# bowang-lab/BioReason

Measured on AMD Instinct MI355X. Metric: GRPO samples/sec (NT-500M+Qwen3-1.7B, DNA 2x1024, prompt 2180, gen 256), higher is better.
Workload: dtype bf16

## Files before the change

bioreason_amd/csrc/k_wgrad.hip:

```cpp
#include "bra_device.h"
#include "bra_api_internal.h"
#include "bra_lora_plan.h"

namespace bra {

struct WgradArgs {
    const bf16_t* Y; long ldy;
    const bf16_t* T; long ldt;
    float* C; long c_sn, c_sr;
    int M, N, R;
    int m_chunk;
    float alpha;
    DropCfg d;
    int nb_live;
};

constexpr int WG_YP = 128 + 8;

template <int RB, int DROP, int NL = RB, int RM = 0, int TR = 32, int NT = NL>
__global__ __launch_bounds__(256) void wgrad_tn_kernel(WgradArgs g) {
    static_assert(!DROP || (NL == (NT * TR + 31) / 32 && NT <= 4), "live blocks = the blocks the targets cover");
    constexpr int NYS = DROP ? NT : 2;
    __shared__ bf16_t ys[NYS][32 * WG_YP];
    constexpr int WG_TP = 32 * RB + 8, TPT = RB >= 2 ? RB / 2 : 1;
    __shared__ bf16_t ts[2][32 * WG_TP];
    const int tid = (int)threadIdx.x, lane = tid & 63, wave = tid >> 6, h = lane >> 5;
    const int n0 = (int)blockIdx.x * 128;
    const int m_lo = (int)blockIdx.y * g.m_chunk;
    int m_hi = m_lo + g.m_chunk;
    m_hi = m_hi < g.M ? m_hi : g.M;
    const int nstep = m_hi > m_lo ? (m_hi - m_lo + 31) / 32 : 0;
    const u32x4 zero4 = {0u, 0u, 0u, 0u};

    const int yr = tid >> 4, yc = (tid & 15) * 8;
    const bool ycol_ok = n0 + yc + 8 <= g.N;
    u32x4 ry[2], rt[TPT];
    auto issue = [&](int s) {
        const int m0 = m_lo + 32 * s;
#pragma unroll
        for (int i = 0; i < 2; ++i) {
            const int m = m0 + yr + 16 * i;
            const int mc = m < g.M ? m : g.M - 1;
            ry[i] = ld16(g.Y + (long)mc * g.ldy + (ycol_ok ? n0 + yc : 0));
        }
#pragma unroll
        for (int i = 0; i < TPT; ++i) {
            const int c = tid + 256 * i, tr = c / (4 * RB), tc = (c % (4 * RB)) * 8;
            const int m = m0 + (tr < 32 ? tr : 0);
            const int mc = m < g.M ? m : g.M - 1;
            rt[i] = ld16(g.T + (long)mc * g.ldt + tc);
        }
    };
    auto commit = [&](int buf, int s) {
        const int m0 = m_lo + 32 * s;
        u32x4 yv[2];
#pragma unroll
        for (int i = 0; i < 2; ++i) yv[i] = (m0 + yr + 16 * i < m_hi && ycol_ok) ? ry[i] : zero4;
        if (DROP) {
#pragma unroll
            for (int i = 0; i < 2; ++i) {
                const uint32_t e0 = (uint32_t)(m_lo + 32 * s + yr + 16 * i) * (uint32_t)g.N + (uint32_t)(n0 + yc);
#pragma unroll
                for (int jt = 0; jt < NT; ++jt)
                    st16(&ys[jt][(yr + 16 * i) * WG_YP + yc], drop_apply8(yv[i], g.d.seed[jt], e0, g.d.thr16, g.d.inv_keep));
            }
        } else {
            st16(&ys[buf][yr * WG_YP + yc], yv[0]);
            st16(&ys[buf][(yr + 16) * WG_YP + yc], yv[1]);
        }
#pragma unroll
        for (int i = 0; i < TPT; ++i) {
            const int c = tid + 256 * i, tr = c / (4 * RB), tc = (c % (4 * RB)) * 8;
            const int m = m0 + (tr < 32 ? tr : 0);
            if (tr < 32) st16(&ts[buf][tr * WG_TP + tc], m < m_hi ? rt[i] : zero4);
        }
    };

    f32x16 acc[RB];
#pragma unroll
    for (int rb = 0; rb < RB; ++rb)
#pragma unroll
        for (int r = 0; r < 16; ++r) acc[rb][r] = 0.f;

    if (nstep > 0) { issue(0); commit(0, 0); }
    __syncthreads();
    const int ncol0 = wave * 32 + (lane & 31);
    constexpr bool r_major = RM != 0;
    for (int s = 0; s < nstep; ++s) {
        const int buf = s & 1;
        issue(s + 1 < nstep ? s + 1 : s);
        sched_fence();
        const int ncol = opaque_i(ncol0);
#pragma unroll
        for (int kk = 0; kk < 2; ++kk) {
            const int mb = 16 * kk + 8 * h;
            u32x4 af0;
            if (!DROP) {
#pragma unroll
                for (int j = 0; j < 4; ++j)
                    af0[j] = (uint32_t)ys[buf][(mb + 2 * j) * WG_YP + ncol] | ((uint32_t)ys[buf][(mb + 2 * j + 1) * WG_YP + ncol] << 16);
            }
            auto y_frag = [&](int jt) {
                u32x4 f;
#pragma unroll
                for (int j = 0; j < 4; ++j)
                    f[j] = (uint32_t)ys[jt][(mb + 2 * j) * WG_YP + ncol] | ((uint32_t)ys[jt][(mb + 2 * j + 1) * WG_YP + ncol] << 16);
                return f;
            };
            auto t_frag = [&](int rb) {
                const int rc = rb * 32 + (lane & 31);
                uint32_t b[4];
#pragma unroll
                for (int j = 0; j < 4; ++j)
                    b[j] = (uint32_t)ts[buf][(mb + 2 * j) * WG_TP + rc] | ((uint32_t)ts[buf][(mb + 2 * j + 1) * WG_TP + rc] << 16);
                const u32x4 bf = {b[0], b[1], b[2], b[3]};
                return bf;
            };
            if constexpr (!DROP || TR == 32) {
#pragma unroll
                for (int rb = 0; rb < NL; ++rb) {
                    u32x4 af = af0;
                    if (DROP) af = y_frag(rb);
                    const u32x4 bf = t_frag(rb);
                    acc[rb] = r_major ? mfma_32x32x16(bf, af, acc[rb]) : mfma_32x32x16(af, bf, acc[rb]);
                }
            } else if constexpr (TR > 32) {
#pragma unroll
                for (int jt = 0; jt < NT; ++jt) {
                    const u32x4 af = y_frag(jt);
#pragma unroll
                    for (int b = 0; b < TR / 32; ++b) {
                        const int rb = jt * (TR / 32) + b;
                        const u32x4 bf = t_frag(rb);
                        acc[rb] = r_major ? mfma_32x32x16(bf, af, acc[rb]) : mfma_32x32x16(af, bf, acc[rb]);
                    }
                }
            } else {
#pragma unroll
                for (int jt = 0; jt < NT; ++jt) {
                    const int rb = jt * TR / 32;
                    const u32x4 af = y_frag(jt);
                    const u32x4 tf = t_frag(rb);
                    const u32x4 bf = (lane & 31) / TR == jt % (32 / TR) ? tf : zero4;
                    acc[rb] = r_major ? mfma_32x32x16(bf, af, acc[rb]) : mfma_32x32x16(af, bf, acc[rb]);
                }
            }
        }
        if (DROP) __syncthreads();
        if (s + 1 < nstep) commit(buf ^ 1, s + 1);
        __syncthreads();
    }
    if (nstep == 0) return;
    if (r_major) {
        const int n = n0 + wave * 32 + (lane & 31);
        float* const cb = g.C + (long)n * g.c_sn + (long)(4 * h) * g.c_sr;
#pragma unroll
        for (int rb = 0; rb < RB; ++rb)
#pragma unroll
            for (int q = 0; q < 16; ++q) {
                const int rq = rb * 32 + (q & 3) + 8 * (q >> 2);
                if (n < g.N && rq + 4 * h < g.R) atomicAdd(cb + (long)rq * g.c_sr, g.alpha * acc[rb][q]);
            }
        return;
    }
    float* const cb = g.C + (long)(n0 + wave * 32 + 4 * h) * g.c_sn + (long)(lane & 31) * g.c_sr;
#pragma unroll
    for (int rb = 0; rb < RB; ++rb) {
        const int r = rb * 32 + (lane & 31);
        if (r >= g.R) continue;
#pragma unroll
        for (int q = 0; q < 16; ++q) {
            const int nq = (q & 3) + 8 * (q >> 2);
            const int n = n0 + wave * 32 + nq + 4 * h;
            if (n < g.N) atomicAdd(cb + (long)nq * g.c_sn + (long)(32 * rb) * g.c_sr, g.alpha * acc[rb][q]);
        }
    }
}

}

using namespace bra;

static int wgrad_launch(WgradArgs& g, int m_chunk, bool drop, const LoraSlice& s, void* stream) {
    if (m_chunk <= 0) {
        const int ntile = (g.N + 127) / 128;
        int splits = (512 + ntile - 1) / ntile;
        m_chunk = (g.M + splits - 1) / splits;
        m_chunk = m_chunk < 256 ? 256 : m_chunk;
    }
    g.m_chunk = (m_chunk + 31) / 32 * 32;
    const dim3 grid((g.N + 127) / 128, (g.M + g.m_chunk - 1) / g.m_chunk);
    bra_stream_t st = (bra_stream_t)stream;
    const bool rm = g.c_sn == 1;
#define BRA_WG(C_, RB_, NL_, TR_, NT_)                                                                             \
    if (C_) {                                                                                                      \
        if (drop && rm) BRA_LAUNCH((wgrad_tn_kernel<RB_, 1, NL_, 1, TR_, NT_>), grid, dim3(256), 0, st, g);        \
        else if (drop) BRA_LAUNCH((wgrad_tn_kernel<RB_, 1, NL_, 0, TR_, NT_>), grid, dim3(256), 0, st, g);         \
        else if (rm) BRA_LAUNCH((wgrad_tn_kernel<RB_, 0, RB_, 1>), grid, dim3(256), 0, st, g);                     \
        else BRA_LAUNCH((wgrad_tn_kernel<RB_, 0, RB_, 0>), grid, dim3(256), 0, st, g);                             \
    } else
    BRA_LORA_ROWS(BRA_WG) return BRA_ERR_ARG;
#undef BRA_WG
    return BRA_LAUNCH_STATUS();
}

static int wgrad_slices(const void* Y, long ldy, const void* T, long ldt, float* C, long c_sn, long c_sr, int M, int N, int R, float alpha,
                        int m_chunk, bool drop, float p, const unsigned* seeds, int r, int nt, void* stream) {
    return lora_for_slices(r, nt, R, [&](LoraSlice s) {
        if (!drop) { s.r = 32; s.nts = s.Rs / 32; }
        WgradArgs g = {(const bf16_t*)Y, ldy, (const bf16_t*)T + s.c0, ldt, C + (long)s.c0 * c_sr, c_sn, c_sr, M, N, s.Rs, 0, alpha,
                       drop ? make_cfg(p, seeds + s.j0, s.nts) : DropCfg{}, 0};
        return wgrad_launch(g, m_chunk, drop, s, stream);
    });
}

extern "C" int bra_wgrad_tn(const void* Y, long ldy, const void* T, long ldt, float* C, long c_sn, long c_sr, int M, int N,
                            int R, float alpha, int m_chunk, void* stream) {
    if (M == 0 || N == 0) return 0;
    if (!Y || !T || !C || M < 0 || N < 0 || N % 8 || ldy % 8 || ldt % 8 || R <= 0 || (R != 32 && R % 64)) return BRA_ERR_ARG;
    return wgrad_slices(Y, ldy, T, ldt, C, c_sn, c_sr, M, N, R, alpha, m_chunk, false, 0.f, nullptr, 0, 0, stream);
}

extern "C" int bra_wgrad_tn_drop(const void* Y, long ldy, const void* T, long ldt, float* C, long c_sn, long c_sr, int M,
                                 int N, int R, float alpha, int m_chunk, float p, unsigned s0, unsigned s1, unsigned s2,
                                 unsigned s3, int r, int nt, void* stream) {
    if (M == 0 || N == 0) return 0;
    if (!Y || !T || !C || M < 0 || N < 0 || N % 8 || ldy % 8 || ldt % 8 || !lora_drop_ok(p, M, N, r, nt, R)) return BRA_ERR_ARG;
    const unsigned seeds[4] = {s0, s1, s2, s3};
    return wgrad_slices(Y, ldy, T, ldt, C, c_sn, c_sr, M, N, R, alpha, m_chunk, true, p, seeds, r, nt, stream);
}
```

bioreason_amd/engine.py:

```python
from __future__ import annotations

import math
from dataclasses import dataclass, field
from typing import Dict, List, Optional, Tuple

import torch

from . import ops
from .arena import TrainableArena

BF16 = torch.bfloat16


def rope_tables(npos: int, hd: int, theta: float, device, round_bf16: bool = True) -> Tuple[torch.Tensor, torch.Tensor]:
    inv = 1.0 / (theta ** (torch.arange(0, hd, 2, dtype=torch.float32) / hd))
    fr = torch.arange(npos, dtype=torch.float32)[:, None] * inv[None, :]
    c, s = fr.cos(), fr.sin()
    if round_bf16:
        c, s = c.to(BF16).float(), s.to(BF16).float()
    return c.contiguous().to(device), s.contiguous().to(device)


class LoraGroup:

# ... 68 lines not shown


def _mix32(a: int, b: int) -> int:
    h = (a * 0x9E3779B1 + b * 0x85EBCA6B + 0x165667B1) & 0xFFFFFFFF
    h ^= h >> 15
    h = (h * 0x2C1B3C6D) & 0xFFFFFFFF
    h ^= h >> 12
    h = (h * 0x297A2D39) & 0xFFFFFFFF
    h ^= h >> 15
    return h


import contextlib as _contextlib
import os as _os
FUSE_SWIGLU = _os.environ.get("BRA_FUSE_SWIGLU", "1") == "1"

_nullctx = _contextlib.nullcontext

LORA_GROUP_INDEX = {"qkv": 0, "o": 1, "gu": 2, "d": 3}


def lora_drop_seeds(pass_seed: int, layer: int, group: str, n_targets: int):
    base = (layer * 4 + LORA_GROUP_INDEX[group]) * 4
    return [_mix32(pass_seed, base + j) for j in range(n_targets)]


class QwenEngine:
    def __init__(self, cfg, device):
        self.cfg = cfg
        self.device = device
        self.H = cfg.hidden_size
        self.Hq, self.Hkv, self.hd = cfg.num_attention_heads, cfg.num_key_value_heads, cfg.head_dim
        self.F = cfg.intermediate_size
        self.L = cfg.num_hidden_layers
        self.V = cfg.vocab_size
        self.eps = cfg.rms_norm_eps
        self.Nq, self.Nkv = self.Hq * self.hd, self.Hkv * self.hd
        self.scale = self.hd ** -0.5
        self.layers: List[QwenLayerW] = [QwenLayerW() for _ in range(self.L)]
        self.norm_w: torch.Tensor = None
        self.E: torch.Tensor = None
        self.ET: Optional[torch.Tensor] = None
        self._rope = None
        self._rope_len = 0
        self.layer_done_hook = None

    def rope(self, npos: int):
        if self._rope is None or self._rope_len < npos:
            n = max(npos, 512)
            theta = self.cfg.rope_parameters["rope_theta"] if hasattr(self.cfg, "rope_parameters") else self.cfg.rope_theta
            self._rope = rope_tables(n, self.hd, theta, self.device)
            self._rope_len = n
        return self._rope

    def ensure_transposed(self):
        for L in self.layers:
            if L.WqkvT is None:
                L.WqkvT = ops.transpose2d(L.Wqkv)
                L.WoT = ops.transpose2d(L.Wo)
                L.WguT = ops.transpose2d(L.Wgu)
                L.WdT = ops.transpose2d(L.Wd)
        if self.ET is None:
            self.ET = ops.transpose2d(self.E)

    SMALL_M = 8192

    @staticmethod
    def _down(x2d, A, scaling, live_rows):
        if x2d.shape[0] < QwenEngine.SMALL_M and A.shape[0] in (32, 64, 128):
            return ops.lora_down_drop(x2d, A, scaling, 0.0, [0] * min(A.shape[0] // 32, (live_rows + 31) // 32), rank=32)
        return ops.gemm_nt(x2d, A, alpha=scaling)

    @staticmethod
    def _lora_fwd(x2d, W, G: Optional[LoraGroup], on: bool, res=None, out=None, drop=None):
        if G is not None and on:
            if drop is not None:
                t = ops.lora_down_drop(x2d, G.A, G.scaling, drop[0], drop[1], drop[2])
            else:
                t = QwenEngine._down(x2d, G.A, G.scaling, len(G.n_sizes) * G.r)
            return ops.gemm_nt(x2d, W, a2=t, b2=G.B, res=res, out=out), t
        return ops.gemm_nt(x2d, W, res=res, out=out), None

    @staticmethod
    def _lora_bwd(dy, WT, G: Optional[LoraGroup], on: bool, x2d, t, drop=None):
        if G is not None and on:
            dts = QwenEngine._down(dy, G.BT, G.scaling, len(G.n_sizes) * G.r)
            if drop is not None:
                dxl = ops.lora_up_drop(dts, G.AT, drop[0], drop[1], drop[2])
                dx = ops.gemm_nt(dy, WT, res=dxl)
            else:
                dx = ops.gemm_nt(dy, WT, a2=dts, b2=G.AT)
            ops.wgrad_tn(dy, t, G.B_grad)
            ops.wgrad_tn(x2d, dts, G.A_grad, transposed_out=True, drop=drop[:2] if drop is not None else None,
                         rank=drop[2] if drop is not None else 32)
            return dx
        return ops.gemm_nt(dy, WT)

    def _drop(self, m: "SeqMeta", li: int, group: str):
        G = self.layers[li].lora[group]
        if G is None or not m.lora_on or m.drop_p <= 0.0:
            return None
        if G.r not in ops.LORA_DROP_RANKS:
            raise NotImplementedError(f"LoRA dropout needs an adapter rank in {list(ops.LORA_DROP_RANKS)} (one mask stream per target "
                                      f"module, built for these ranks), not r = {G.r}")
        return (m.drop_p, lora_drop_seeds(m.drop_seed, li, group, len(G.n_sizes)), G.r)

    def use_fp8(self, W8):
        eng = self

        class _Ctx:
            def __enter__(self_):
                self_.prev = getattr(eng, "_fp8", None)
                eng._fp8 = W8

            def __exit__(self_, *a):
                eng._fp8 = self_.prev
        return _Ctx()

    def fp8_supported(self) -> bool:
        return self.H % 128 == 0 and self.F % 128 == 0 and self.Nq % 128 == 0

    def fp8_weight_images(self, merged=None):
        out = []
        for li, L in enumerate(self.layers):
            W = merged[li] if merged is not None else {"Wqkv": L.Wqkv, "Wo": L.Wo, "Wgu": L.Wgu, "Wd": L.Wd}
            out.append({"Wqkv": ops.quant_rows_fp8(W["Wqkv"], colw=L.ln1), "Wo": ops.quant_rows_fp8(W["Wo"]),
                        "Wgu": ops.quant_rows_fp8(W["Wgu"], colw=L.ln2), "Wd": ops.quant_rows_fp8(W["Wd"])})
        return out

    def _layer_fwd_fp8(self, li: int, x: torch.Tensor, m: SeqMeta, kv_out, R):
        L = self.layers[li]
        B, S, T = m.B, m.S, m.B * m.S
        cosT, sinT = self.rope(m.max_pos or m.S)
        xq, xs = ops.quant_rows_fp8(x, rms_eps=self.eps)
        qkv = ops.gemm_fp8_nt(xq, xs, R["Wqkv"][0], R["Wqkv"][1])
        q = torch.empty((B, S, self.Hq, self.hd), dtype=BF16, device=x.device)
        if kv_out is None:
            k = torch.empty((B, S, self.Hkv, self.hd), dtype=BF16, device=x.device)
            v = torch.empty((B, S, self.Hkv, self.hd), dtype=BF16, device=x.device)
            s_off = 0
        else:
            kc, vc, s_off = kv_out[:3]
            k, v = kc.permute(0, 2, 1, 3), vc.permute(0, 2, 1, 3)
        ops.qk_norm_rope_fwd(qkv, L.qn, L.kn, cosT, sinT, m.pos, S, self.Hq, self.Hkv, self.hd, self.eps, 1.0, q, k, v, s_off)
        if kv_out is not None:
            k, v = k[:, :s_off + S], v[:, :s_off + S]
        vt = ops.head_transpose(v)
        if kv_out is not None and len(kv_out) > 3 and kv_out[3] is not None:
            kv_out[3].append(vt)
        o, _ = ops.attn_fwd(q, k, vt, m.kmask, True, self.scale, need_lse=False)
        oq, os_ = ops.quant_rows_fp8(o.view(T, self.Nq))
        h = ops.gemm_fp8_nt(oq, os_, R["Wo"][0], R["Wo"][1], res=x)
        hq, hs = ops.quant_rows_fp8(h, rms_eps=self.eps)
        gu = ops.gemm_fp8_nt(hq, hs, R["Wgu"][0], R["Wgu"][1])
        aq, as_ = ops.swiglu_quant_fp8(gu)
        return ops.gemm_fp8_nt(aq, as_, R["Wd"][0], R["Wd"][1], res=h)

    def layer_fwd(self, li: int, x: torch.Tensor, m: SeqMeta, save: bool, kv_out=None):
        w8 = getattr(self, "_fp8", None)
        if w8 is not None and not save:
            return self._layer_fwd_fp8(li, x, m, kv_out, w8[li]), None
        L = self.layers[li]
        B, S, T = m.B, m.S, m.B * m.S
        cosT, sinT = self.rope(m.max_pos or m.S)
        xn = ops.rmsnorm_fwd(x, L.ln1, self.eps)
        qkv, t1 = self._lora_fwd(xn, L.Wqkv, L.lora["qkv"], m.lora_on, drop=self._drop(m, li, "qkv"))
        q = torch.empty((B, S, self.Hq, self.hd), dtype=BF16, device=x.device)
        if kv_out is None:
            k = torch.empty((B, S, self.Hkv, self.hd), dtype=BF16, device=x.device)
            v = torch.empty((B, S, self.Hkv, self.hd), dtype=BF16, device=x.device)
            s_off = 0
        else:
            kc, vc, s_off = kv_out[:3]
            k, v = kc.permute(0, 2, 1, 3), vc.permute(0, 2, 1, 3)
        ops.qk_norm_rope_fwd(qkv, L.qn, L.kn, cosT, sinT, m.pos, S, self.Hq, self.Hkv, self.hd, self.eps, 1.0, q, k, v, s_off)
        if kv_out is not None:
            k, v = k[:, :s_off + S], v[:, :s_off + S]
        vt = ops.head_transpose(v)
        if kv_out is not None and len(kv_out) > 3 and kv_out[3] is not None:
            kv_out[3].append(vt)
        o, lse = ops.attn_fwd(q, k, vt, m.kmask, True, self.scale, need_lse=save)
        o2 = o.view(T, self.Nq)
        h, t2 = self._lora_fwd(o2, L.Wo, L.lora["o"], m.lora_on, res=x, drop=self._drop(m, li, "o"))
        hn = ops.rmsnorm_fwd(h, L.ln2, self.eps)
        gu = t3 = act = None
        if not save and FUSE_SWIGLU:
            G3, d3 = L.lora["gu"], self._drop(m, li, "gu")
            if G3 is not None and m.lora_on:
                t3 = ops.lora_down_drop(hn, G3.A, G3.scaling, d3[0], d3[1], d3[2]) if d3 is not None else self._down(hn, G3.A, G3.scaling, len(G3.n_sizes) * G3.r)
                act = ops.gemm_swiglu(hn, L.Wgu, a2=t3, b2=G3.B)
            else:
                act = ops.gemm_swiglu(hn, L.Wgu)
        if act is None:
            if t3 is not None:
                gu = ops.gemm_nt(hn, L.Wgu, a2=t3, b2=L.lora["gu"].B)
            else:
                gu, t3 = self._lora_fwd(hn, L.Wgu, L.lora["gu"], m.lora_on, drop=self._drop(m, li, "gu"))
            act = ops.swiglu_fwd(gu)
        y, t4 = self._lora_fwd(act, L.Wd, L.lora["d"], m.lora_on, res=h, drop=self._drop(m, li, "d"))
        saved = (x, xn, t1, qkv, q, k, v, o, lse, t2, h, hn, t3, gu, act, t4) if save else None
        return y, saved

    def layer_bwd(self, li: int, dy: torch.Tensor, saved, m: SeqMeta, prefix: int = 0, extra_dkv=None):
        L = self.layers[li]
        (x, xn, t1, qkv, q, k, v, o, lse, t2, h, hn, t3, gu, act, t4) = saved
        B, S, T = m.B, m.S, m.B * m.S
        cosT, sinT = self.rope(m.max_pos or m.S)
        on = m.lora_on
        dact = self._lora_bwd(dy, L.WdT, L.lora["d"], on, act, t4, drop=self._drop(m, li, "d"))
        dgu = ops.swiglu_bwd(gu, dact)
        dhn = self._lora_bwd(dgu, L.WguT, L.lora["gu"], on, hn, t3, drop=self._drop(m, li, "gu"))
        dh = ops.rmsnorm_bwd(dhn, h, L.ln2, self.eps, dres=dy)
        do = self._lora_bwd(dh, L.WoT, L.lora["o"], on, o.view(T, self.Nq), t2, drop=self._drop(m, li, "o"))
        dq, dk, dv = ops.attn_bwd(q, k, v, o, do.view(B, S, self.Hq, self.hd), lse, m.kmask, True, self.scale)
        pre = None
        if prefix > 0:
            pre = (dk[:, :prefix], dv[:, :prefix])
            dk, dv = dk[:, prefix:], dv[:, prefix:]
        if extra_dkv is not None:
            dk = ops.group_sum(extra_dkv[0], extra_dkv[2], add=dk)
            dv = ops.group_sum(extra_dkv[1], extra_dkv[2], add=dv)
        dqkv = ops.qk_norm_rope_bwd(qkv, L.qn, L.kn, cosT, sinT, m.pos, S, self.Hq, self.Hkv, self.hd, self.eps, 1.0, dq, dk, dv)
        dxn = self._lora_bwd(dqkv, L.WqkvT, L.lora["qkv"], on, xn, t1, drop=self._drop(m, li, "qkv"))
        dx = ops.rmsnorm_bwd(dxn, x, L.ln1, self.eps, dres=dh)
        return (dx, pre) if prefix > 0 else dx

    def forward_hidden(self, x: torch.Tensor, m: SeqMeta, save: bool):
        tape = []
        for li in range(self.L):
            x, saved = self.layer_fwd(li, x, m, save)
            tape.append(saved)
        hid = ops.rmsnorm_fwd(x, self.norm_w, self.eps)
        return hid, (tape, x) if save else None

    def backward_hidden(self, dhid: torch.Tensor, tape_x, m: SeqMeta):
        tape, xlast = tape_x
        dx = ops.rmsnorm_bwd(dhid, xlast, self.norm_w, self.eps)
        for li in reversed(range(self.L)):
            dx = self.layer_bwd(li, dx, tape[li], m)
            tape[li] = None
            if self.layer_done_hook is not None:
                self.layer_done_hook(li)
        return dx


    def forward_hidden_shared(self, xp: torch.Tensor, mp: SeqMeta, xc: torch.Tensor, mc: SeqMeta, copies: int, save: bool, side=None):
        R, P, B, C = mp.B, mp.S, mc.B, mc.S
        assert B == R * copies
        dev = xp.device
        tape_p, tape_c = [], []
        main = torch.cuda.current_stream(dev) if side is not None else None
        if side is not None:
            side.wait_stream(main)
            xc.record_stream(side)
        for li in range(self.L):
            kc_r = torch.empty((R, self.Hkv, P, self.hd), dtype=BF16, device=dev)
            vc_r = torch.empty((R, self.Hkv, P, self.hd), dtype=BF16, device=dev)
            xp, sp = self.layer_fwd(li, xp, mp, save, kv_out=(kc_r, vc_r, 0))
            tape_p.append(sp)
            if side is not None:
                ev = torch.cuda.Event()
                ev.record(main)
                kc_r.record_stream(side)
                vc_r.record_stream(side)
            with (torch.cuda.stream(side) if side is not None else _nullctx()):
                if side is not None:
                    side.wait_event(ev)
                kc = torch.empty((B, self.Hkv, P + C, self.hd), dtype=BF16, device=dev)
                vc = torch.empty((B, self.Hkv, P + C, self.hd), dtype=BF16, device=dev)
                ops.group_broadcast(kc_r, kc, copies)
                ops.group_broadcast(vc_r, vc, copies)
                xc, sc = self.layer_fwd(li, xc, mc, save, kv_out=(kc, vc, P))
                tape_c.append(sc)
        last = torch.arange(R, device=dev, dtype=torch.int32) * P + (P - 1)
        xp_last = ops.gather_rows(last, xp)
        hid_last = ops.rmsnorm_fwd(xp_last, self.norm_w, self.eps)
        with (torch.cuda.stream(side) if side is not None else _nullctx()):
            hid_c = ops.rmsnorm_fwd(xc, self.norm_w, self.eps)
        if side is not None:
            main.wait_stream(side)
            for t_ in (hid_c, xc):
                t_.record_stream(main)
        return hid_last, hid_c, ((tape_p, tape_c, xp_last, xc, last) if save else None)

    def backward_hidden_shared(self, dhid_last: torch.Tensor, dhid_c: torch.Tensor, tape, mp: SeqMeta, mc: SeqMeta, copies: int, side=None):
        tape_p, tape_c, xp_last, xc, last = tape
        dev = dhid_c.device
        main = torch.cuda.current_stream(dev) if side is not None else None
        if side is not None:
            side.wait_stream(main)
            dhid_c.record_stream(side)
        with (torch.cuda.stream(side) if side is not None else _nullctx()):
            dxc = ops.rmsnorm_bwd(dhid_c, xc, self.norm_w, self.eps)
        dxp = ops.scatter_rows(last, ops.rmsnorm_bwd(dhid_last, xp_last, self.norm_w, self.eps), mp.B * mp.S)
        for li in reversed(range(self.L)):
            with (torch.cuda.stream(side) if side is not None else _nullctx()):
                dxc, pre = self.layer_bwd(li, dxc, tape_c[li], mc, prefix=mp.S)
                tape_c[li] = None
                if side is not None:
                    ev = torch.cuda.Event()
                    ev.record(side)
            if side is not None:
                main.wait_event(ev)
                pre[0].record_stream(main)
                pre[1].record_stream(main)
            dxp = self.layer_bwd(li, dxp, tape_p[li], mp, extra_dkv=(pre[0], pre[1], copies))
            tape_p[li] = None
# ... 72 lines not shown
```

bioreason_amd/ops.py:

```python
from __future__ import annotations

import math
import os
from typing import Optional, Tuple

import torch

from ._lib import current_stream, get_lib

BF16 = torch.bfloat16


def _ld(t: torch.Tensor) -> int:
    assert t.stride(-1) == 1, "last dim must be contiguous"
    return t.stride(-2) if t.dim() >= 2 else t.shape[-1]


def _rows(t: torch.Tensor) -> int:
    return t.numel() // t.shape[-1]


def _as2d(t: torch.Tensor) -> torch.Tensor:
    return t.reshape(-1, t.shape[-1]) if t.dim() != 2 else t


def gemm_nt(
    a: torch.Tensor,
    b: torch.Tensor,
    *,
    a2: Optional[torch.Tensor] = None,
    b2: Optional[torch.Tensor] = None,
    bias: Optional[torch.Tensor] = None,
    res: Optional[torch.Tensor] = None,
    out: Optional[torch.Tensor] = None,
    alpha: float = 1.0,
    out_f32: bool = False,
    accumulate: bool = False,
) -> torch.Tensor:
    a = _as2d(a)
    M, K = a.shape
    N = b.shape[0]
    assert b.shape[1] == K and a.dtype == BF16 and b.dtype == BF16
    K2 = 0
    if a2 is not None:
        a2 = _as2d(a2)
        K2 = a2.shape[1]
        assert b2 is not None and b2.shape == (N, K2) and a2.shape[0] == M
    if out is None:
        out = torch.empty((M, N), dtype=torch.float32 if out_f32 else BF16, device=a.device)
    else:
        assert out.shape == (M, N) and out.dtype == (torch.float32 if out_f32 else BF16)
    if res is not None:
        res = _as2d(res)
        assert res.shape == (M, N) and res.dtype == BF16
    prof = GEMM_PROFILE
    timed = prof is not None and a.is_cuda and prof.wants(M, N, K, K2)
    if timed:
        e0 = torch.cuda.Event(enable_timing=True)
        e0.record()
    get_lib().call(
        "bra_gemm_bf16_nt", a, _ld(a), b, _ld(b), a2, _ld(a2) if a2 is not None else 0, b2,
        _ld(b2) if b2 is not None else 0, K2, out, _ld(out), M, N, K, alpha, bias, res,
        _ld(res) if res is not None else 0, int(out_f32), int(accumulate), current_stream(a),
    )
    if timed:
        e1 = torch.cuda.Event(enable_timing=True)
        e1.record()
        nbytes = 2.0 * (M * K + N * K + (M + N) * K2 + (M * N if res is not None else 0)) + M * N * (4.0 if out_f32 else 2.0)
        prof.records.append((2.0 * M * N * (K + K2), e0, e1, nbytes, (M, N, K, K2, res is not None)))
    return out


class GemmProfile:

    def __init__(self, min_m: int = 1024, dominant_only: bool = True):
        self.min_m = min_m
        self.dominant_only = dominant_only
        self.records = []

    def wants(self, M: int, N: int, K: int, K2: int) -> bool:
        if not self.dominant_only:
            return M >= self.min_m
        if K % 64 or K2 % 64:
            return False
        t = ((M + 255) // 256) * ((N + 255) // 256)
        rounds = (t + 255) // 256
        if t >= 140 and (t <= 256 or 100 * t >= 75 * rounds * 256):
            return True
        if ((M + 255) // 256) * ((N + 127) // 128) >= 128:
            return True
        return ((M + 127) // 128) * ((N + 127) // 128) >= 128

    def summary(self):
        torch.cuda.synchronize()
        fl = sum(r[0] for r in self.records)
        ms = sum(r[1].elapsed_time(r[2]) for r in self.records)
        n = len(self.records)
        by = sum(r[3] for r in self.records)
        return {"launches": n, "flops": fl, "ms": ms, "avg_launch_ms": ms / max(n, 1), "tflops": fl / max(ms, 1e-9) / 1e9,
                "flops_per_launch": fl / max(n, 1), "bytes_per_launch": by / max(n, 1)}


def gemm_profile_by_shape(prof: "GemmProfile"):
    torch.cuda.synchronize()
    agg = {}
    for r in prof.records:
        a = agg.setdefault(r[4], [0, 0.0, 0.0])
        a[0] += 1
        a[1] += r[1].elapsed_time(r[2])
        a[2] += r[0]
    return sorted(((k, n, ms, fl / max(ms, 1e-9) / 1e9) for k, (n, ms, fl) in agg.items()), key=lambda t: -t[2])


GEMM_PROFILE: Optional[GemmProfile] = None


def gemm_nt_splitk(a: torch.Tensor, b: torch.Tensor, out: torch.Tensor, alpha: float = 1.0, split_k: int = 0) -> torch.Tensor:
    M, K = a.shape
    N = b.shape[0]
    assert b.shape[1] == K and out.shape == (M, N) and out.dtype == torch.float32
    if split_k <= 0:
        tiles = ((M + 127) // 128) * ((N + 127) // 128)
        split_k = max(1, min(K // 256 if K >= 256 else 1, (512 + tiles - 1) // tiles))
    get_lib().call("bra_gemm_bf16_nt_splitk", a, _ld(a), b, _ld(b), out, _ld(out), M, N, K, alpha, split_k, current_stream(a))
    return out


def wgrad_tn(y: torch.Tensor, t: torch.Tensor, out: torch.Tensor, transposed_out: bool = False, alpha: float = 1.0,
             m_chunk: int = 0, drop=None, rank: int = 32) -> torch.Tensor:
    M, N = y.shape
    R = t.shape[1]
    assert t.shape[0] == M and out.dtype == torch.float32 and out.shape == ((R, N) if transposed_out else (N, R))
    c_sn, c_sr = (1, _ld(out)) if transposed_out else (_ld(out), 1)
    if drop is not None:
        get_lib().call("bra_wgrad_tn_drop", y, _ld(y), t, _ld(t), out, c_sn, c_sr, M, N, R, alpha, m_chunk, drop[0],
                       *_group(drop[1], rank, R), current_stream(y))
        return out
    get_lib().call("bra_wgrad_tn", y, _ld(y), t, _ld(t), out, c_sn, c_sr, M, N, R, alpha, m_chunk, current_stream(y))
    return out


LORA_DROP_RANKS = (8, 16, 32, 64, 128)


def _group(seeds, rank, R):
    if rank not in LORA_DROP_RANKS:
        raise NotImplementedError(f"LoRA dropout is built for adapter ranks {list(LORA_DROP_RANKS)}, not r = {rank}")
    if rank == 32:
        seeds = seeds[:max(R // 32, 1)]
    elif not 1 <= len(seeds) <= 3:
        raise ValueError(f"a fused LoRA group has 1 to 3 targets, got {len(seeds)} seeds")
    s = [int(x) & 0xFFFFFFFF for x in seeds]
    return (*(s + [0, 0, 0, 0])[:4], rank, len(s))


def dropout_mask(M: int, K: int, p: float, seed: int, device) -> torch.Tensor:
    out = torch.empty((M, K), dtype=torch.uint8, device=device)
    get_lib().call("bra_dropout_mask", out, M, K, p, int(seed) & 0xFFFFFFFF, current_stream(out))
    return out


LORA_DOWN_SPLITK = os.environ.get("BRA_LORA_SPLITK", "1") != "0"


def lora_down_drop(x: torch.Tensor, A: torch.Tensor, alpha: float, p: float, seeds, rank: int = 32) -> torch.Tensor:
    M, K = x.shape
    R = A.shape[0]
    t = torch.empty((M, R), dtype=BF16, device=x.device)
    lib = get_lib()
    ks = int(lib._dll.bra_lora_down_splitk_plan(int(M), int(K))) if LORA_DOWN_SPLITK else 1
    part = torch.empty((ks, M, R), dtype=torch.float32, device=x.device) if ks > 1 else None
    lib.call("bra_lora_down_drop", x, _ld(x), A, _ld(A), t, _ld(t), M, K, R, alpha, p, *_group(seeds, rank, R), part, ks,
             current_stream(x))
    return t


def lora_up_drop(dts: torch.Tensor, AT: torch.Tensor, p: float, seeds, rank: int = 32) -> torch.Tensor:
    M, R = dts.shape
    K = AT.shape[0]
    out = torch.empty((M, K), dtype=BF16, device=dts.device)
    get_lib().call("bra_lora_up_drop", dts, _ld(dts), AT, _ld(AT), out, _ld(out), M, K, R, p, *_group(seeds, rank, R),
                   current_stream(dts))
    return out


def lmhead_logprob(h: torch.Tensor, emb: torch.Tensor, tgt: torch.Tensor) -> Tuple[torch.Tensor, torch.Tensor]:
    M, K = h.shape
    V = emb.shape[0]
    nchunk = (V + 63) // 64
    dev = h.device
    pm = torch.empty((M, nchunk), dtype=torch.float32, device=dev)
    ps = torch.empty((M, nchunk), dtype=torch.float32, device=dev)
    tl = torch.zeros((M,), dtype=torch.float32, device=dev)
    lse = torch.empty((M,), dtype=torch.float32, device=dev)
    logp = torch.empty((M,), dtype=torch.float32, device=dev)
    st = current_stream(h)
    lib = get_lib()
    lib.call("bra_lmhead_lse_partials", h, _ld(h), emb, _ld(emb), M, V, K, tgt, pm, ps, tl, st)
    lib.call("bra_lse_merge", pm, ps, tl, lse, logp, M, nchunk, st)
    return logp, lse


def lmhead_dlogits(h: torch.Tensor, emb: torch.Tensor, tgt: torch.Tensor, lse: torch.Tensor, coef: torch.Tensor) -> torch.Tensor:
    M, K = h.shape
    V = emb.shape[0]
    out = torch.empty((M, V), dtype=BF16, device=h.device)
    get_lib().call("bra_lmhead_dlogits", h, _ld(h), emb, _ld(emb), M, V, K, tgt, lse, coef, out, _ld(out), current_stream(h))
    return out


def rmsnorm_fwd(x: torch.Tensor, w: torch.Tensor, eps: float) -> torch.Tensor:
    x2 = _as2d(x)
    y = torch.empty_like(x2)
    get_lib().call("bra_rmsnorm_fwd", x2, _ld(x2), w, y, _ld(y), None, x2.shape[0], x2.shape[1], eps, current_stream(x))
    return y.view(x.shape)


def rmsnorm_bwd(dy: torch.Tensor, x: torch.Tensor, w: torch.Tensor, eps: float, dres: Optional[torch.Tensor] = None) -> torch.Tensor:
    x2, dy2 = _as2d(x), _as2d(dy)
    dx = torch.empty_like(x2)
    d2 = _as2d(dres) if dres is not None else None
    get_lib().call("bra_rmsnorm_bwd", dy2, _ld(dy2), x2, _ld(x2), w, d2, _ld(d2) if d2 is not None else 0, dx, _ld(dx),
                   x2.shape[0], x2.shape[1], eps, current_stream(x))
    return dx.view(x.shape)


# ... 485 lines not shown
```

include/bioreason_hip.h:

```cpp
#ifndef BIOREASON_HIP_H
#define BIOREASON_HIP_H
#ifdef __cplusplus
extern "C" {
#endif

#define BRA_ERR_ARG (-1)
#define BRA_ERR_UNSUPPORTED (-2)

int bra_gemm_bf16_nt(const void* A, long lda, const void* B, long ldb, const void* A2, long lda2, const void* B2,
                     long ldb2, int K2, void* C, long ldc, int M, int N, int K, float alpha, const void* bias,
                     const void* res, long ldres, int out_f32, int accumulate, void* stream);

int bra_gemm_bf16_nt_splitk(const void* A, long lda, const void* B, long ldb, void* C, long ldc, int M, int N, int K,
                            float alpha, int split_k, void* stream);

int bra_wgrad_tn(const void* Y, long ldy, const void* T, long ldt, float* C, long c_sn, long c_sr, int M, int N, int R,
                 float alpha, int m_chunk, void* stream);

int bra_lora_down_splitk_plan(int M, int K);
int bra_lora_down_drop(const void* x, long ldx, const void* A, long lda, void* t, long ldt, int M, int K, int R, float alpha,
                       float p, unsigned s0, unsigned s1, unsigned s2, unsigned s3, int r, int nt, float* part, int ksplit,
                       void* stream);
int bra_lora_up_drop(const void* dts, long ldd, const void* AT, long ldat, void* out, long ldo, int M, int K, int R, float p,
                     unsigned s0, unsigned s1, unsigned s2, unsigned s3, int r, int nt, void* stream);
int bra_wgrad_tn_drop(const void* Y, long ldy, const void* T, long ldt, float* C, long c_sn, long c_sr, int M, int N, int R,
                      float alpha, int m_chunk, float p, unsigned s0, unsigned s1, unsigned s2, unsigned s3, int r, int nt,
                      void* stream);
int bra_dropout_mask(void* out, int M, int K, float p, unsigned seed, void* stream);

int bra_lmhead_lse_partials(const void* H, long ldh, const void* E, long lde, int M, int V, int K, const int* tgt,
                            float* part_max, float* part_sum, float* tgt_logit, void* stream);
int bra_lse_merge(const float* part_max, const float* part_sum, const float* tgt_logit, float* lse, float* logp,
                  int rows, int nchunk, void* stream);
int bra_lmhead_dlogits(const void* H, long ldh, const void* E, long lde, int M, int V, int K, const int* tgt,
                       const float* lse, const float* coef, void* dlogits, long ldd, void* stream);

int bra_rmsnorm_fwd(const void* x, long ldx, const void* w, void* y, long ldy, float* rstd, int rows, int cols,
                    float eps, void* stream);
int bra_rmsnorm_bwd(const void* dy, long lddy, const void* x, long ldx, const void* w, const void* dres, long lddres,
                    void* dx, long lddx, int rows, int cols, float eps, void* stream);
int bra_layernorm_fwd(const void* x, long ldx, const void* w, const void* b, void* y, long ldy, int rows, int cols,
                      float eps, void* stream);
int bra_swiglu_fwd(const void* gu, long ldgu, void* act, long ldact, int rows, int F, void* stream);
int bra_swiglu_bwd(const void* gu, long ldgu, const void* dact, long lddact, void* dgu, long lddgu, int rows, int F,
                   void* stream);
int bra_qk_norm_rope_fwd(const void* qkv, long ldqkv, const void* qw, const void* kw, const float* cosT,
                         const float* sinT, const int* pos, int T, int S, int Hq, int Hkv, int hd, float eps,
                         float qscale, void* q, long q_sb, long q_ss, long q_sh, void* k, long k_sb, long k_ss,
                         long k_sh, void* v, long v_sb, long v_ss, long v_sh, int s_off, void* stream);
int bra_qk_norm_rope_bwd(const void* qkv, long ldqkv, const void* qw, const void* kw, const float* cosT,
                         const float* sinT, const int* pos, int T, int S, int Hq, int Hkv, int hd, float eps,
                         float qscale, const void* dq, long q_sb, long q_ss, long q_sh, const void* dk, long k_sb,
                         long k_ss, long k_sh, const void* dv, long v_sb, long v_ss, long v_sh, void* dqkv,
                         long lddqkv, void* stream);

int bra_attn_fwd(const void* q, long q_sb, long q_ss, long q_sh, const void* k, long k_sb, long k_ss, long k_sh,
                 const void* vt, long vt_sb, long vt_sh, long vt_sd, void* o, long o_sb, long o_ss, long o_sh,
                 float* lse, const void* kmask, int B, int Hq, int Hkv, int Sq, int Sk, int hd, int causal,
                 int q_off, float scale, void* stream);
int bra_attn_fwd_split(const void* q, long q_sb, long q_ss, long q_sh, const void* k, long k_sb, long k_ss, long k_sh,
                       const void* vt, long vt_sb, long vt_sh, long vt_sd, void* o, long o_sb, long o_ss, long o_sh,
                       float* lse, const void* kmask, int B, int Hq, int Hkv, int Sq, int Sk, int hd, int causal,
                       int q_off, float scale, int nsplit, float* part_o, float* part_ml, void* stream);
int bra_attn_bwd(const void* q, long q_sb, long q_ss, long q_sh, const void* k, long k_sb, long k_ss, long k_sh,
                 const void* v, long v_sb, long v_ss, long v_sh, const void* dout, long do_sb, long do_ss, long do_sh,
                 const void* kt, long kt_sb, long kt_sh, long kt_sd, const void* qt, long qt_sb, long qt_sh,
                 long qt_sd, const void* dot, long dot_sb, long dot_sh, long dot_sd, const float* lse,
                 const float* delta, const void* kmask, void* dq, long dq_sb, long dq_ss, long dq_sh, void* dk,
                 long dk_sb, long dk_ss, long dk_sh, void* dv, long dv_sb, long dv_ss, long dv_sh, int B, int Hq,
                 int Hkv, int Sq, int Sk, int hd, int causal, int q_off, float scale, void* stream);
int bra_attn_bwd_split(const void* q, long q_sb, long q_ss, long q_sh, const void* k, long k_sb, long k_ss, long k_sh,
                 const void* v, long v_sb, long v_ss, long v_sh, const void* dout, long do_sb, long do_ss, long do_sh,
                 const void* kt, long kt_sb, long kt_sh, long kt_sd, const void* qt, long qt_sb, long qt_sh,
                 long qt_sd, const void* dot, long dot_sb, long dot_sh, long dot_sd, const float* lse,
                 const float* delta, const void* kmask, void* dq, long dq_sb, long dq_ss, long dq_sh, void* dk,
                 long dk_sb, long dk_ss, long dk_sh, void* dv, long dv_sb, long dv_ss, long dv_sh, int B, int Hq,
                 int Hkv, int Sq, int Sk, int hd, int causal, int q_off, float scale, int nsplit_dq, float* part_dq, int nsplit_kv, float* part_dk, float* part_dv, void* stream);
int bra_attn_decode_nchunk(int len);
int bra_attn_decode(const void* q, const void* kc, const void* vc, const void* kmask, float* part_o, float* part_ml,
                    void* o, int B, int Hq, int Hkv, int hd, int Smax, int len, float scale, void* stream);

int bra_qwen_layer_desc_size(void);
int bra_qwen_decode_step(const void* layers_host, int L, int B, int H, int Hq, int Hkv, int hd, int F, int Smax,
                         float eps, float scale, const void* E, const void* norm_w, const float* cosT,
                         const float* sinT, const int* tok, const int* pos, const void* kmask, int cur_len,
                         int lora_on, void* x, void* xn, void* qkv, void* q, void* o, void* h, void* hn, void* gu,
                         void* act, void* t, float* part_o, float* part_ml, void* hid, void* stream);

int bra_dec_gemm(const void* x, long ldx, const void* norm_w, float eps, const void* W, long ldw, const void* res,
                 long ldres, void* out, long ldo, int M, int N, int K, int act, int out_f32, void* stream);
int bra_dec_attn_partial(const void* qkv, long ldqkv, const void* qw, const void* kw, const float* cosT,
                         const float* sinT, const int* pos, void* kc, void* vc, const void* kmask, float* part_o,
                         float* part_ml, int B, int Hq, int Hkv, int hd, int Smax, int cur_len, float eps, float scale,
                         int chunk_off, int nchunk_tot, const int* t_dev, void* stream);
int bra_dec_gemm2(const void* x, long ldx, const float* ss_in, int nss_in, const void* norm_w, float eps, const void* W,
                  long ldw, const void* res, long ldres, void* out, long ldo, float* ss_out, int nss_out, int M, int N,
                  int K, int act, int out_f32, void* stream);
int bra_dec_gemm2_packed(const void* x, long ldx, const float* ss_in, int nss_in, const void* norm_w, float eps, const void* W,
                         long ldw, const void* res, long ldres, void* out, long ldo, float* ss_out, int nss_out, int M, int N,
                         int K, int act, int out_f32, int packed, void* stream);
int bra_dec_pack_weights_fp8(const void* W, long ldw, int N, int K, int act, int out_f32, const void* norm_w, void* out_q,
                             float* out_scale, void* stream);
int bra_dec_gemm2_fp8(const void* x, long ldx, const float* ss_in, int nss_in, float eps, const void* Wq, const float* wscale,
                      const void* res, long ldres, void* out, long ldo, float* ss_out, int nss_out, int M, int N, int K, int act,
                      int out_f32, int norm_folded, void* stream);
int bra_gemm_swiglu_bf16_nt(const void* A, long lda, const void* W, long ldw, const void* A2, long lda2, const void* B2, long ldb2, int K2,
                            void* C, long ldc, int M, int F, int K, float alpha, void* stream);
int bra_quant_rows_fp8(const void* x, long ldx, int M, int K, const void* colw, void* q, long ldq, float* scale, int rms, float eps,
                       void* stream);
int bra_swiglu_quant_fp8(const void* gu, long ldgu, int M, int F, void* q, long ldq, float* scale, void* stream);
int bra_gemm_fp8_nt(const void* A8, long lda, const float* sa, const void* B8, long ldb, const float* sb, void* C, long ldc, int M, int N,
// ... 111 lines not shown
```

Before: 19.64.

## Batch per-layer LoRA weight-gradient GEMMs into one grouped kernel launch

Adds a grouped wgrad kernel that runs up to eight LoRA weight-gradient problems in a single launch. Each block finds its problem from a prefix-sum table and dispatches to the matching template instance through a switch. The per-layer backward now collects the A/B gradient problems for the d, gu, o and qkv projections and launches them together at the end of the layer. This aims to cut launch overhead and let small wgrad grids share the GPU. The cost is delayed gradient work, LDS sized for the largest instance (which may lower occupancy), and a Python fallback path to single launches.

```diff
diff --git a/bioreason_amd/csrc/k_wgrad.hip b/bioreason_amd/csrc/k_wgrad.hip
--- a/bioreason_amd/csrc/k_wgrad.hip
+++ b/bioreason_amd/csrc/k_wgrad.hip
@@ -1,6 +1,7 @@
 #include "bra_device.h"
 #include "bra_api_internal.h"
 #include "bra_lora_plan.h"
+#include "../../include/bioreason_hip.h"
 
 namespace bra {
 
@@ -17,16 +18,19 @@
 
 constexpr int WG_YP = 128 + 8;
 
+template <int RB, int DROP, int NT>
+constexpr int wgrad_lds_elems() { return (DROP ? NT : 2) * 32 * WG_YP + 2 * 32 * (32 * RB + 8); }
+
 template <int RB, int DROP, int NL = RB, int RM = 0, int TR = 32, int NT = NL>
-__global__ __launch_bounds__(256) void wgrad_tn_kernel(WgradArgs g) {
+__device__ __forceinline__ void wgrad_tn_body(const WgradArgs& g, bf16_t* lds, int bx, int by) {
     static_assert(!DROP || (NL == (NT * TR + 31) / 32 && NT <= 4), "live blocks = the blocks the targets cover");
     constexpr int NYS = DROP ? NT : 2;
-    __shared__ bf16_t ys[NYS][32 * WG_YP];
+    bf16_t (*ys)[32 * WG_YP] = reinterpret_cast<bf16_t (*)[32 * WG_YP]>(lds);
     constexpr int WG_TP = 32 * RB + 8, TPT = RB >= 2 ? RB / 2 : 1;
-    __shared__ bf16_t ts[2][32 * WG_TP];
+    bf16_t (*ts)[32 * WG_TP] = reinterpret_cast<bf16_t (*)[32 * WG_TP]>(lds + NYS * 32 * WG_YP);
     const int tid = (int)threadIdx.x, lane = tid & 63, wave = tid >> 6, h = lane >> 5;
-    const int n0 = (int)blockIdx.x * 128;
-    const int m_lo = (int)blockIdx.y * g.m_chunk;
+    const int n0 = bx * 128;
+    const int m_lo = by * g.m_chunk;
     int m_hi = m_lo + g.m_chunk;
     m_hi = m_hi < g.M ? m_hi : g.M;
     const int nstep = m_hi > m_lo ? (m_hi - m_lo + 31) / 32 : 0;
@@ -177,11 +181,52 @@
     }
 }
 
+template <int RB, int DROP, int NL = RB, int RM = 0, int TR = 32, int NT = NL>
+__global__ __launch_bounds__(256) void wgrad_tn_kernel(WgradArgs g) {
+    __shared__ __attribute__((aligned(16))) bf16_t lds[wgrad_lds_elems<RB, DROP, NT>()];
+    wgrad_tn_body<RB, DROP, NL, RM, TR, NT>(g, lds, (int)blockIdx.x, (int)blockIdx.y);
+}
+
+#define BRA_WGRAD_GROUP_INSTS(X) X(0, 2, 0, 2, 0, 2) X(1, 2, 1, 1, 1, 1) X(2, 2, 1, 2, 1, 2) X(3, 4, 1, 3, 1, 3) X(4, 4, 0, 4, 0, 4)
+
+constexpr int WG_GROUP_MAX = 8;
+struct WgradGroupArgs {
+    WgradArgs g[WG_GROUP_MAX];
+    int end[WG_GROUP_MAX];
+    int inst[WG_GROUP_MAX];
+};
+
+constexpr int wgrad_group_lds_elems() {
+    int m = 0;
+#define BRA_WG_LDS(ID_, RB_, DROP_, NL_, RM_, NT_) m = wgrad_lds_elems<RB_, DROP_, NT_>() > m ? wgrad_lds_elems<RB_, DROP_, NT_>() : m;
+    BRA_WGRAD_GROUP_INSTS(BRA_WG_LDS)
+#undef BRA_WG_LDS
+    return m;
+}
+
+__global__ __launch_bounds__(256) void wgrad_group_kernel(WgradGroupArgs a) {
+    __shared__ __attribute__((aligned(16))) bf16_t lds[wgrad_group_lds_elems()];
+    const int b = (int)blockIdx.x;
+    int p = 0, first = 0;
+#pragma unroll
+    for (int i = 0; i < WG_GROUP_MAX - 1; ++i)
+        if (b >= a.end[i]) { p = i + 1; first = a.end[i]; }
+    const WgradArgs& g = a.g[p];
+    const int ntile = (g.N + 127) / 128, local = b - first;
+    const int bx = local % ntile, by = local / ntile;
+    switch (a.inst[p]) {
+#define BRA_WG_CASE(ID_, RB_, DROP_, NL_, RM_, NT_) case ID_: wgrad_tn_body<RB_, DROP_, NL_, RM_, 32, NT_>(g, lds, bx, by); break;
+        BRA_WGRAD_GROUP_INSTS(BRA_WG_CASE)
+#undef BRA_WG_CASE
+        default: break;
+    }
+}
+
 }
 
 using namespace bra;
 
-static int wgrad_launch(WgradArgs& g, int m_chunk, bool drop, const LoraSlice& s, void* stream) {
+static dim3 wgrad_grid(WgradArgs& g, int m_chunk) {
     if (m_chunk <= 0) {
         const int ntile = (g.N + 127) / 128;
         int splits = (512 + ntile - 1) / ntile;
@@ -189,7 +234,11 @@
         m_chunk = m_chunk < 256 ? 256 : m_chunk;
     }
     g.m_chunk = (m_chunk + 31) / 32 * 32;
-    const dim3 grid((g.N + 127) / 128, (g.M + g.m_chunk - 1) / g.m_chunk);
+    return dim3((g.N + 127) / 128, (g.M + g.m_chunk - 1) / g.m_chunk);
+}
+
+static int wgrad_launch(WgradArgs& g, int m_chunk, bool drop, const LoraSlice& s, void* stream) {
+    const dim3 grid = wgrad_grid(g, m_chunk);
     bra_stream_t st = (bra_stream_t)stream;
     const bool rm = g.c_sn == 1;
 #define BRA_WG(C_, RB_, NL_, TR_, NT_)                                                                             \
@@ -204,20 +253,43 @@
     return BRA_LAUNCH_STATUS();
 }
 
-static int wgrad_slices(const void* Y, long ldy, const void* T, long ldt, float* C, long c_sn, long c_sr, int M, int N, int R, float alpha,
-                        int m_chunk, bool drop, float p, const unsigned* seeds, int r, int nt, void* stream) {
+template <class F>
+static int wgrad_for_slices(const void* Y, long ldy, const void* T, long ldt, float* C, long c_sn, long c_sr, int M, int N, int R,
+                            float alpha, bool drop, float p, const unsigned* seeds, int r, int nt, F&& f) {
     return lora_for_slices(r, nt, R, [&](LoraSlice s) {
         if (!drop) { s.r = 32; s.nts = s.Rs / 32; }
         WgradArgs g = {(const bf16_t*)Y, ldy, (const bf16_t*)T + s.c0, ldt, C + (long)s.c0 * c_sr, c_sn, c_sr, M, N, s.Rs, 0, alpha,
                        drop ? make_cfg(p, seeds + s.j0, s.nts) : DropCfg{}, 0};
-        return wgrad_launch(g, m_chunk, drop, s, stream);
+        return f(g, s);
     });
+}
+
+static int wgrad_slices(const void* Y, long ldy, const void* T, long ldt, float* C, long c_sn, long c_sr, int M, int N, int R, float alpha,
+                        int m_chunk, bool drop, float p, const unsigned* seeds, int r, int nt, void* stream) {
+    return wgrad_for_slices(Y, ldy, T, ldt, C, c_sn, c_sr, M, N, R, alpha, drop, p, seeds, r, nt,
+                            [&](WgradArgs& g, const LoraSlice& s) { return wgrad_launch(g, m_chunk, drop, s, stream); });
+}
+
+static bool wgrad_args_ok(const void* Y, long ldy, const void* T, long ldt, const float* C, int M, int N) {
+    return Y && T && C && M >= 0 && N >= 0 && N % 8 == 0 && ldy % 8 == 0 && ldt % 8 == 0;
+}
+
+static int wgrad_group_inst(bool drop, bool rm, const LoraSlice& s) {
+    int RB = 0, NL = 0, TR = 0, NT = 0;
+#define BRA_WG(C_, RB_, NL_, TR_, NT_) if (C_) { RB = RB_; NL = NL_; TR = TR_; NT = NT_; } else
+    BRA_LORA_ROWS(BRA_WG) return -1;
+#undef BRA_WG
+    if (!drop) { NL = NT = RB; TR = 32; }
+#define BRA_WG_ID(ID_, RB_, DROP_, NL_, RM_, NT_) if (RB == RB_ && drop == (DROP_ != 0) && NL == NL_ && rm == (RM_ != 0) && TR == 32 && NT == NT_) return ID_;
+    BRA_WGRAD_GROUP_INSTS(BRA_WG_ID)
+#undef BRA_WG_ID
+    return -1;
 }
 
 extern "C" int bra_wgrad_tn(const void* Y, long ldy, const void* T, long ldt, float* C, long c_sn, long c_sr, int M, int N,
                             int R, float alpha, int m_chunk, void* stream) {
     if (M == 0 || N == 0) return 0;
-    if (!Y || !T || !C || M < 0 || N < 0 || N % 8 || ldy % 8 || ldt % 8 || R <= 0 || (R != 32 && R % 64)) return BRA_ERR_ARG;
+    if (!wgrad_args_ok(Y, ldy, T, ldt, C, M, N) || R <= 0 || (R != 32 && R % 64)) return BRA_ERR_ARG;
     return wgrad_slices(Y, ldy, T, ldt, C, c_sn, c_sr, M, N, R, alpha, m_chunk, false, 0.f, nullptr, 0, 0, stream);
 }
 
@@ -225,7 +297,48 @@
                                  int N, int R, float alpha, int m_chunk, float p, unsigned s0, unsigned s1, unsigned s2,
                                  unsigned s3, int r, int nt, void* stream) {
     if (M == 0 || N == 0) return 0;
-    if (!Y || !T || !C || M < 0 || N < 0 || N % 8 || ldy % 8 || ldt % 8 || !lora_drop_ok(p, M, N, r, nt, R)) return BRA_ERR_ARG;
+    if (!wgrad_args_ok(Y, ldy, T, ldt, C, M, N) || !lora_drop_ok(p, M, N, r, nt, R)) return BRA_ERR_ARG;
     const unsigned seeds[4] = {s0, s1, s2, s3};
     return wgrad_slices(Y, ldy, T, ldt, C, c_sn, c_sr, M, N, R, alpha, m_chunk, true, p, seeds, r, nt, stream);
 }
+
+static_assert(sizeof(bra_wgrad_problem) == 104, "the host layer packs this struct (bioreason_amd/ops.py)");
+
+extern "C" int bra_wgrad_tn_group(const bra_wgrad_problem* problems, int n, void* stream) {
+    if (n < 0 || (n > 0 && !problems)) return BRA_ERR_ARG;
+    WgradGroupArgs a;
+    int cnt = 0;
+    auto flush = [&]() {
+        int total = 0;
+        for (int i = 0; i < cnt; ++i) {
+            const dim3 grid = wgrad_grid(a.g[i], a.g[i].m_chunk);
+            total += (int)(grid.x * grid.y);
+            a.end[i] = total;
+        }
+        if (total > 0) {
+            for (int i = cnt; i < WG_GROUP_MAX; ++i) { a.g[i] = WgradArgs{}; a.end[i] = total; a.inst[i] = 0; }
+            BRA_LAUNCH(wgrad_group_kernel, dim3((unsigned)total), dim3(256), 0, (bra_stream_t)stream, a);
+        }
+        cnt = 0;
+        return BRA_LAUNCH_STATUS();
+    };
+    for (int pass = 0; pass < 2; ++pass) {
+        for (int i = 0; i < n; ++i) {
+            const bra_wgrad_problem& q = problems[i];
+            if (q.M == 0 || q.N == 0) continue;
+            const bool drop = q.nt > 0;
+            if (pass == 0 && (!wgrad_args_ok(q.Y, q.ldy, q.T, q.ldt, q.C, q.M, q.N) || q.nt < 0 ||
+                              (drop ? !lora_drop_ok(q.p, q.M, q.N, q.r, q.nt, q.R) : (q.R <= 0 || (q.R != 32 && q.R % 64)))))
+                return BRA_ERR_ARG;
+            const int rc = wgrad_for_slices(q.Y, q.ldy, q.T, q.ldt, q.C, q.c_sn, q.c_sr, q.M, q.N, q.R, q.alpha, drop, q.p, q.seed, q.r, q.nt,
+                                            [&](WgradArgs& g, const LoraSlice& s) {
+                const int id = wgrad_group_inst(drop, g.c_sn == 1, s);
+                if (pass == 0) return id < 0 ? BRA_ERR_UNSUPPORTED : 0;
+                a.g[cnt] = g; a.g[cnt].m_chunk = q.m_chunk; a.inst[cnt] = id;
+                return ++cnt == WG_GROUP_MAX ? flush() : 0;
+            });
+            if (rc) return rc;
+        }
+    }
+    return flush();
+}
diff --git a/bioreason_amd/engine.py b/bioreason_amd/engine.py
--- a/bioreason_amd/engine.py
+++ b/bioreason_amd/engine.py
@@ -174,7 +174,7 @@
         return ops.gemm_nt(x2d, W, res=res, out=out), None
 
     @staticmethod
-    def _lora_bwd(dy, WT, G: Optional[LoraGroup], on: bool, x2d, t, drop=None):
+    def _lora_bwd(dy, WT, G: Optional[LoraGroup], on: bool, x2d, t, drop=None, pending: Optional[list] = None):
         if G is not None and on:
             dts = QwenEngine._down(dy, G.BT, G.scaling, len(G.n_sizes) * G.r)
             if drop is not None:
@@ -182,9 +182,13 @@
                 dx = ops.gemm_nt(dy, WT, res=dxl)
             else:
                 dx = ops.gemm_nt(dy, WT, a2=dts, b2=G.AT)
-            ops.wgrad_tn(dy, t, G.B_grad)
-            ops.wgrad_tn(x2d, dts, G.A_grad, transposed_out=True, drop=drop[:2] if drop is not None else None,
-                         rank=drop[2] if drop is not None else 32)
+            wg = (ops.wgrad_problem(dy, t, G.B_grad),
+                  ops.wgrad_problem(x2d, dts, G.A_grad, transposed_out=True, drop=drop[:2] if drop is not None else None,
+                                    rank=drop[2] if drop is not None else 32))
+            if pending is not None:
+                pending.extend(wg)
+            else:
+                ops.wgrad_tn_group(wg)
             return dx
         return ops.gemm_nt(dy, WT)
 
@@ -299,11 +303,12 @@
         B, S, T = m.B, m.S, m.B * m.S
         cosT, sinT = self.rope(m.max_pos or m.S)
         on = m.lora_on
-        dact = self._lora_bwd(dy, L.WdT, L.lora["d"], on, act, t4, drop=self._drop(m, li, "d"))
+        wg = []
+        dact = self._lora_bwd(dy, L.WdT, L.lora["d"], on, act, t4, drop=self._drop(m, li, "d"), pending=wg)
         dgu = ops.swiglu_bwd(gu, dact)
-        dhn = self._lora_bwd(dgu, L.WguT, L.lora["gu"], on, hn, t3, drop=self._drop(m, li, "gu"))
+        dhn = self._lora_bwd(dgu, L.WguT, L.lora["gu"], on, hn, t3, drop=self._drop(m, li, "gu"), pending=wg)
         dh = ops.rmsnorm_bwd(dhn, h, L.ln2, self.eps, dres=dy)
-        do = self._lora_bwd(dh, L.WoT, L.lora["o"], on, o.view(T, self.Nq), t2, drop=self._drop(m, li, "o"))
+        do = self._lora_bwd(dh, L.WoT, L.lora["o"], on, o.view(T, self.Nq), t2, drop=self._drop(m, li, "o"), pending=wg)
         dq, dk, dv = ops.attn_bwd(q, k, v, o, do.view(B, S, self.Hq, self.hd), lse, m.kmask, True, self.scale)
         pre = None
         if prefix > 0:
@@ -313,8 +318,9 @@
             dk = ops.group_sum(extra_dkv[0], extra_dkv[2], add=dk)
             dv = ops.group_sum(extra_dkv[1], extra_dkv[2], add=dv)
         dqkv = ops.qk_norm_rope_bwd(qkv, L.qn, L.kn, cosT, sinT, m.pos, S, self.Hq, self.Hkv, self.hd, self.eps, 1.0, dq, dk, dv)
-        dxn = self._lora_bwd(dqkv, L.WqkvT, L.lora["qkv"], on, xn, t1, drop=self._drop(m, li, "qkv"))
+        dxn = self._lora_bwd(dqkv, L.WqkvT, L.lora["qkv"], on, xn, t1, drop=self._drop(m, li, "qkv"), pending=wg)
         dx = ops.rmsnorm_bwd(dxn, x, L.ln1, self.eps, dres=dh)
+        ops.wgrad_tn_group(wg)
         return (dx, pre) if prefix > 0 else dx
 
     def forward_hidden(self, x: torch.Tensor, m: SeqMeta, save: bool):
diff --git a/bioreason_amd/ops.py b/bioreason_amd/ops.py
--- a/bioreason_amd/ops.py
+++ b/bioreason_amd/ops.py
@@ -1,7 +1,9 @@
 from __future__ import annotations
 
+import ctypes
 import math
 import os
+import struct
 from typing import Optional, Tuple
 
 import torch
@@ -142,6 +144,62 @@
 
 LORA_DROP_RANKS = (8, 16, 32, 64, 128)
 
+_WGRAD_PROBLEM = struct.Struct("PqPqPqqiiififIIIIii")
+_WGRAD_GROUP_REFUSED = set()
+
+
+def wgrad_problem(y: torch.Tensor, t: torch.Tensor, out: torch.Tensor, transposed_out: bool = False, alpha: float = 1.0,
+                  m_chunk: int = 0, drop=None, rank: int = 32):
+    return (y, t, out, transposed_out, alpha, m_chunk, drop, rank)
+
+
+def _wgrad_key(pr):
+    return (bool(pr[3]), len(pr[6][1]) if pr[6] is not None else 0, pr[7], pr[1].shape[1])
+
+
+def _wgrad_pack(pr) -> bytes:
+    y, t, out, transposed_out, alpha, m_chunk, drop, rank = pr
+    M, N = y.shape
+    R = t.shape[1]
+    assert t.shape[0] == M and out.dtype == torch.float32 and out.shape == ((R, N) if transposed_out else (N, R))
+    c_sn, c_sr = (1, _ld(out)) if transposed_out else (_ld(out), 1)
+    p, grp = (drop[0], _group(drop[1], rank, R)) if drop is not None else (0.0, (0, 0, 0, 0, 0, 0))
+    return _WGRAD_PROBLEM.pack(y.data_ptr(), _ld(y), t.data_ptr(), _ld(t), out.data_ptr(), c_sn, c_sr, M, N, R, alpha, m_chunk, p, *grp)
+
+
+def wgrad_tn_group(problems) -> list:
+    routes = ["group"] * len(problems)
+    if not problems:
+        return routes
+    lib = get_lib()
+    if not lib.emulated and not all(pr[0].is_cuda for pr in problems):
+        raise RuntimeError("bra_wgrad_tn_group: a CPU tensor; the HIP library needs device memory")
+    stream = current_stream(problems[0][0])
+
+    def launch(idx):
+        buf = ctypes.create_string_buffer(b"".join(_wgrad_pack(problems[i]) for i in idx))
+        return lib.call_rc("bra_wgrad_tn_group", ctypes.addressof(buf), len(idx), stream)
+
+    def single(i):
+        y, t, out, transposed_out, alpha, m_chunk, drop, rank = problems[i]
+        wgrad_tn(y, t, out, transposed_out, alpha, m_chunk, drop, rank)
+        routes[i] = "single"
+
+    idx = []
+    for i, pr in enumerate(problems):
+        if _wgrad_key(pr) in _WGRAD_GROUP_REFUSED:
+            single(i)
+        else:
+            idx.append(i)
+    if idx and launch(idx) != 0:
+        for i in idx:
+            if launch([i]) != 0:
+                _WGRAD_GROUP_REFUSED.add(_wgrad_key(problems[i]))
+                single(i)
+            else:
+                routes[i] = "group1"
+    return routes
+
 
 def _group(seeds, rank, R):
     if rank not in LORA_DROP_RANKS:
diff --git a/include/bioreason_hip.h b/include/bioreason_hip.h
--- a/include/bioreason_hip.h
+++ b/include/bioreason_hip.h
@@ -27,6 +27,19 @@
                       float alpha, int m_chunk, float p, unsigned s0, unsigned s1, unsigned s2, unsigned s3, int r, int nt,
                       void* stream);
 int bra_dropout_mask(void* out, int M, int K, float p, unsigned seed, void* stream);
+
+typedef struct bra_wgrad_problem {
+    const void* Y; long ldy;
+    const void* T; long ldt;
+    float* C; long c_sn, c_sr;
+    int M, N, R;
+    float alpha;
+    int m_chunk;
+    float p;
+    unsigned seed[4];
+    int r, nt;
+} bra_wgrad_problem;
+int bra_wgrad_tn_group(const bra_wgrad_problem* problems, int n, void* stream);
 
 int bra_lmhead_lse_partials(const void* H, long ldh, const void* E, long lde, int M, int V, int K, const int* tgt,
                             float* part_max, float* part_sum, float* tgt_logit, void* stream);
```

Result: no change. 19.70 (median of 6 runs) (+0.3%).
